# TXH-mercury/VALOR

Hardware: AMD Instinct MI355X
Metric: pretrain samples/sec (V+A+T clip) (higher is better)
Workload: dtype bf16

## Files before the change

valor_amd/csrc/gemm8q.hip:

```cpp
#include "gemm_common.h"
#include <stdlib.h>

#define HT_BYTES 16384
#define BUF_BYTES (4 * HT_BYTES)
#define OFF_A0 0
#define OFF_A1 HT_BYTES
#define OFF_B0 (2 * HT_BYTES)
#define OFF_B1 (3 * HT_BYTES)

template <bool KSLOW> struct FragSet;
template <> struct FragSet<false> { bf16x8_t f[4][2]; };
template <> struct FragSet<true> { TrPair f[4][2]; };
DEVINL bf16x8_t frag_of(const bf16x8_t& f) { return f; }
DEVINL bf16x8_t frag_of(const TrPair& t) { return tr_frag(t); }
DEVINL void mfma_acc(f32x4_t& c, bf16x8_t a, bf16x8_t b) { asm("v_mfma_f32_16x16x32_bf16 %0, %1, %2, %0" : "+a"(c) : "v"(a), "v"(b)); }
DEVINL void mfma_rowsum(f32x4_t& r0, f32x4_t& r1, bf16x8_t ones, bf16x8_t f0, bf16x8_t f1, bf16x8_t f2, bf16x8_t f3, int sel) {
    asm volatile("s_cmp_lt_i32 %7, 1\n\ts_cbranch_scc1 2f\n\ts_cmp_eq_u32 %7, 1\n\ts_cbranch_scc0 1f\n\t"
                 "v_mfma_f32_16x16x32_bf16 %0, %2, %3, %0\n\tv_mfma_f32_16x16x32_bf16 %1, %2, %4, %1\n\ts_branch 2f\n"
                 "1:\n\tv_mfma_f32_16x16x32_bf16 %0, %2, %5, %0\n\tv_mfma_f32_16x16x32_bf16 %1, %2, %6, %1\n"
                 "2:"
                 : "+v"(r0), "+v"(r1) : "v"(ones), "v"(f0), "v"(f1), "v"(f2), "v"(f3), "s"(sel) : "scc");
}
DEVINL void wait8(FragSet<false>&) { asm volatile("s_waitcnt lgkmcnt(0)" ::: "memory"); }
DEVINL void wait8(FragSet<true>& s) { tr_wait8(s.f); }
DEVINL void wait4(FragSet<false>&, int) { asm volatile("s_waitcnt lgkmcnt(0)" ::: "memory"); }
DEVINL void wait4(FragSet<true>& s, int kk) { tr_wait_4(s.f[0][kk], s.f[1][kk], s.f[2][kk], s.f[3][kk]); }

template <bool TA, bool TB>
__global__ __launch_bounds__(256) void gemm_8q_kernel(GemmArgs p) {
    typedef bf16_t T;
    constexpr int BK = 64;
    extern __shared__ __attribute__((aligned(16))) char smem[];

    const int tid = threadIdx.x;
    const int lane = tid & 63;
    const int wave = __builtin_amdgcn_readfirstlane(tid >> 6);
    const int wm = wave >> 1, wn = wave & 1;
    const int fr = lane & 15, fg = lane >> 4;

    const int tiles_n = (p.N + 255) >> 8;
    const int tiles_m = (p.M + 255) >> 8;
    int logical, slice = 0;
    if (p.kslices > 1) {
        const int ntiles = tiles_m * tiles_n;
        const int item = xcd_remap(blockIdx.x, ntiles * p.kslices);
        slice = item / ntiles;
        logical = item - slice * ntiles;
    } else {
        logical = xcd_remap(blockIdx.x, tiles_m * tiles_n);
    }
    int tm = logical / tiles_n, tn = logical - tm * tiles_n;
    if (p.raster_g > 0 && p.kslices <= 1) {
        const int G = p.raster_g, per = G * tiles_m;
        const int grp = logical / per, w = logical - grp * per;
        const int gw = min(G, tiles_n - grp * G);
        tm = w / gw;
        tn = grp * G + (w - tm * gw);
    }
    const int m0 = tm << 8, n0 = tn << 8;

    const int nk_total = p.K / BK;
    int ks_begin = 0, ks_end = nk_total;
    if (p.kslices > 1) {
        ks_begin = slice * p.ksteps_per_slice;
        ks_end = ks_begin + p.ksteps_per_slice;
        if (ks_end > nk_total) ks_end = nk_total;
        if (ks_begin > nk_total) ks_begin = nk_total;
    }
    const int k_first = ks_begin * BK;
    const int ntile = ks_end - ks_begin;

    f32x4_t acc[8][8];
#pragma unroll
    for (int i = 0; i < 8; ++i)
#pragma unroll
        for (int j = 0; j < 8; ++j) acc[i][j] = (f32x4_t){0.f, 0.f, 0.f, 0.f};

    const bool do_rs = TA && p.rowsum_out != nullptr && tn == 0;
    f32x4_t racc[2][2];
#pragma unroll
    for (int i = 0; i < 2; ++i)
#pragma unroll
        for (int j = 0; j < 2; ++j) racc[i][j] = (f32x4_t){0.f, 0.f, 0.f, 0.f};
    bf16x8_t ones = __builtin_bit_cast(bf16x8_t, (u32x4_t){0x3f803f80u, 0x3f803f80u, 0x3f803f80u, 0x3f803f80u});
    asm volatile("" : "+v"(ones));
    const int rs_sel = __builtin_amdgcn_readfirstlane(do_rs ? wn + 1 : 0);

    int oA[2][4], oB[2][4];
    int stepA, stepB;
    {
        const int ldA_b = (int)(p.lda * 2), ldB_b = (int)(p.ldb * 2);
#pragma unroll
        for (int hf = 0; hf < 2; ++hf)
#pragma unroll
            for (int i = 0; i < 4; ++i) {
                const int pc = wave * 4 + i;
                if constexpr (!TA) {
                    const int r = pc * 8 + (lane >> 3), c = (lane & 7) ^ ((lane >> 3) & 7);
                    oA[hf][i] = (m0 + hf * 128 + r) * ldA_b + (k_first + c * 8) * 2;
                } else {
                    const int k = pc * 4 + (lane >> 4), s = lane & 15;
                    const int ic = ((s - 2 * (k & 3) - 8 * ((k >> 3) & 1)) & 15) * 8;
                    oA[hf][i] = (k_first + k) * ldA_b + (m0 + hf * 128 + ic) * 2;
                }
                if constexpr (!TB) {
                    const int r = pc * 8 + (lane >> 3), c = (lane & 7) ^ ((lane >> 3) & 7);
                    oB[hf][i] = (n0 + hf * 128 + r) * ldB_b + (k_first + c * 8) * 2;
                } else {
                    const int k = pc * 4 + (lane >> 4), s = lane & 15;
                    const int ic = ((s - 2 * (k & 3) - 8 * ((k >> 3) & 1)) & 15) * 8;
                    oB[hf][i] = (k_first + k) * ldB_b + (n0 + hf * 128 + ic) * 2;
                }
            }
        stepA = TA ? BK * ldA_b : BK * 2;
        stepB = TB ? BK * ldB_b : BK * 2;
    }
    auto dmaA = [&](int hf, char* buf, int t, int i) {
        const rsrc_t rs = make_rsrc(p.A, t < ntile ? p.bytesA : 0u);
        glds16(rs, buf + (hf ? OFF_A1 : OFF_A0) + wave * 4096 + i * 1024, oA[hf][i]);
        oA[hf][i] += stepA; asm volatile("" : "+v"(oA[hf][i]));
    };
    auto dmaB = [&](int hf, char* buf, int t, int i) {
        const rsrc_t rs = make_rsrc(p.B, t < ntile ? p.bytesB : 0u);
        glds16(rs, buf + (hf ? OFF_B1 : OFF_B0) + wave * 4096 + i * 1024, oB[hf][i]);
        oB[hf][i] += stepB; asm volatile("" : "+v"(oB[hf][i]));
    };

    int trA[4], trB[4];
    {
        const int base = (8 * fg + (fr >> 2)) * 256 + 8 * (fr & 1);
        const int rot = 2 * (fr >> 2) + 8 * (fg & 1);
#pragma unroll
        for (int i = 0; i < 4; ++i) {
            trA[i] = base + 16 * ((2 * (wm * 4 + i) + ((fr >> 1) & 1) + rot) & 15);
            trB[i] = base + 16 * ((2 * (wn * 4 + i) + ((fr >> 1) & 1) + rot) & 15);
        }
    }
    auto rdA = [&](const char* img, FragSet<TA>& s, int mt, int kk) {
        if constexpr (TA) tr_issue(s.f[mt][kk], img + trA[mt] + kk * (32 * 256));
        else s.f[mt][kk] = read_frag<T>(img, wm * 64 + mt * 16 + fr, kk * 4 + fg);
    };
    auto rdB = [&](const char* img, FragSet<TB>& s, int nt, int kk) {
        if constexpr (TB) tr_issue(s.f[nt][kk], img + trB[nt] + kk * (32 * 256));
        else s.f[nt][kk] = read_frag<T>(img, wn * 64 + nt * 16 + fr, kk * 4 + fg);
    };
#define PIN() __builtin_amdgcn_sched_barrier(0)
    auto quadrant = [&](int mh, int nh, FragSet<TA>& sa, FragSet<TB>& sb, auto&& slot) __attribute__((always_inline)) {
#pragma unroll
        for (int kk = 0; kk < 2; ++kk)
#pragma unroll
            for (int mt = 0; mt < 4; ++mt)
#pragma unroll
                for (int nt = 0; nt < 4; ++nt) {
                    const int i = kk * 16 + mt * 4 + nt;
                    mfma_acc(acc[mh * 4 + mt][nh * 4 + nt], frag_of(sb.f[nt][kk]), frag_of(sa.f[mt][kk]));
                    slot(i);
                    PIN();
                }
    };
    auto rowsum = [&](int hh, FragSet<TA>& sa) __attribute__((always_inline)) {
        if constexpr (TA) {
#pragma unroll
            for (int kk = 0; kk < 2; ++kk)
                mfma_rowsum(racc[hh][0], racc[hh][1], ones, frag_of(sa.f[0][kk]), frag_of(sa.f[1][kk]), frag_of(sa.f[2][kk]), frag_of(sa.f[3][kk]), rs_sel);
            PIN();
        }
    };
#define PHASE_END()                                                                                               \
    do {                                                                                                          \
        asm volatile("s_waitcnt vmcnt(20)" ::: "memory");                                                         \
        __builtin_amdgcn_s_barrier();                                                                             \
        PIN();                                                                                                    \
    } while (0)

    FragSet<TA> fax, fay;
    FragSet<TB> fb0, fb1;
    if (ntile > 0) {
#pragma unroll
        for (int t = 0; t < 2; ++t) {
            char* const b = smem + t * BUF_BYTES;
#pragma unroll
            for (int i = 0; i < 4; ++i) dmaA(0, b, t, i);
#pragma unroll
            for (int i = 0; i < 4; ++i) dmaB(0, b, t, i);
#pragma unroll
            for (int i = 0; i < 4; ++i) dmaB(1, b, t, i);
#pragma unroll
            for (int i = 0; i < 4; ++i) dmaA(1, b, t, i);
        }
        PIN();
        PHASE_END();
#pragma unroll
        for (int i = 0; i < 8; ++i) rdA(smem + OFF_A0, fax, i & 3, i >> 2);
#pragma unroll
        for (int i = 0; i < 4; ++i) rdB(smem + OFF_B0, fb0, i, 0);
        PIN();
        wait8(fax); wait4(fb0, 0);
        __builtin_amdgcn_s_barrier();
        PIN();
        for (int rel = 0; rel < ntile; ++rel) {
            char* const cur = smem + (rel & 1) * BUF_BYTES;
            char* const nxt = smem + ((rel & 1) ^ 1) * BUF_BYTES;
            quadrant(0, 0, fax, fb0, [&](int i) {
                if (i < 4) rdB(cur + OFF_B0, fb0, i, 1);
                else if (i < 8) dmaA(0, cur, rel + 2, i - 4);
                else if (i == 15) { PIN(); wait4(fb0, 1); }
                else if (i >= 16 && i < 24) rdB(cur + OFF_B1, fb1, i & 3, (i - 16) >> 2);
            });
            rowsum(0, fax);
            PIN();
            wait8(fb1);
            PHASE_END();
            quadrant(0, 1, fax, fb1, [&](int i) {
                if (i < 8) rdA(cur + OFF_A1, fay, i & 3, i >> 2);
                else if (i < 16 && !(i & 1)) dmaB(0, cur, rel + 2, (i - 8) >> 1);
            });
            PIN();
            wait8(fay);
            PHASE_END();
            quadrant(1, 1, fay, fb1, [&](int i) {
                if (i < 4) rdA(nxt + OFF_A0, fax, i, 0);
                else if (i >= 8 && i < 16 && !(i & 1)) dmaB(1, cur, rel + 2, (i - 8) >> 1);
            });
            rowsum(1, fay);
            PIN();
            wait4(fax, 0);
            PHASE_END();
            quadrant(1, 0, fay, fb0, [&](int i) {
                if (i < 4) rdA(nxt + OFF_A0, fax, i, 1);
                else if (i >= 8 && i < 16 && !(i & 1)) dmaA(1, cur, rel + 2, (i - 8) >> 1);
                else if (i >= 16 && i < 20) rdB(nxt + OFF_B0, fb0, i - 16, 0);
            });
            PIN();
            wait4(fax, 1); wait4(fb0, 0);
            PHASE_END();
        }
    }
    asm volatile("s_nop 15\n\ts_nop 15\n\ts_waitcnt vmcnt(0)" ::: "memory");
    PIN();
    __syncthreads();
#undef PHASE_END
#undef PIN
    if (do_rs && fg == 0) {
#pragma unroll
        for (int hh = 0; hh < 2; ++hh)
#pragma unroll
            for (int i = 0; i < 2; ++i) {
                const int m = m0 + hh * 128 + wm * 64 + (2 * wn + i) * 16 + fr;
                if (m < p.M) {
                    if (p.kslices > 1) p.rowsum_ws[(int64_t)slice * p.M + m] = racc[hh][i][0];
                    else rowsum_store<T>(p, m, racc[hh][i][0]);
                }
            }
    }

    float* sC = (float*)smem;
    float* wsl = p.kslices > 1 ? p.ws + (int64_t)slice * p.M * p.N : nullptr;
    const f32x4_t bias0 = load_bias4<T>(p, n0 + (tid & 31) * 8), bias1 = load_bias4<T>(p, n0 + (tid & 31) * 8 + 4);
#pragma unroll
    for (int pass = 0; pass < 2; ++pass) {
        if (pass) __syncthreads();
#pragma unroll
        for (int mt = 0; mt < 4; ++mt)
#pragma unroll
            for (int ni = 0; ni < 8; ++ni) {
                const int ml = wm * 64 + mt * 16 + fr;
                const int ch = ((ni >> 2) * 32 + wn * 16 + (ni & 3) * 4 + fg) ^ (ml & 7);
                *(f32x4_t*)(sC + ml * 256 + ch * 4) = acc[pass * 4 + mt][ni];
            }
        __syncthreads();
#pragma unroll 2
        for (int it = 0; it < 16; ++it) {
            const int ml = it * 8 + (tid >> 5);
            const int c8 = tid & 31;
            const f32x4_t v0 = *(const f32x4_t*)(sC + ml * 256 + (((2 * c8) ^ (ml & 7)) << 2));
            const f32x4_t v1 = *(const f32x4_t*)(sC + ml * 256 + (((2 * c8 + 1) ^ (ml & 7)) << 2));
            const int m = m0 + pass * 128 + ml, n = n0 + c8 * 8;
            if (wsl) {
                splitk_store8(p, slice, m, n, v0, v1);
            } else {
                epilogue_store8<true, 0>(p, m, n, v0, v1, bias0, bias1);
            }
        }
    }
}

void launch_gemm_8q(hipStream_t st, int transA, int transB, const GemmArgs& p_in) {
    GemmArgs p = p_in;
    p.fast_epi = 0;
    p.raster_g = 0;
    p.st_mode = 0;
    const int tiles = ((p.M + 255) / 256) * ((p.N + 255) / 256);
    dim3 grid(tiles * (p.kslices > 1 ? p.kslices : 1));
    const size_t lds = 2 * BUF_BYTES;
#define VALOR_8Q_LAUNCH(TA_, TB_)                                                                               \
    do {                                                                                                        \
        static bool attr_set = false;                                                                           \
        if (!attr_set) {                                                                                        \
            hipFuncSetAttribute((const void*)gemm_8q_kernel<TA_, TB_>, hipFuncAttributeMaxDynamicSharedMemorySize, (int)lds); \
            attr_set = true;                                                                                    \
        }                                                                                                       \
        hipLaunchKernelGGL((gemm_8q_kernel<TA_, TB_>), grid, dim3(256), lds, st, p);                            \
    } while (0)
    if (transA && transB) VALOR_8Q_LAUNCH(true, true);
    else if (!transA && !transB) VALOR_8Q_LAUNCH(false, false);
    else if (!transA && transB) VALOR_8Q_LAUNCH(false, true);
    else VALOR_8Q_LAUNCH(true, false);
#undef VALOR_8Q_LAUNCH
}
```

Baseline: 580.6.

## Add slot-scheduled main loop for TA&&TB GEMM with finer LDS waits

For the transposed-A and transposed-B instantiation, replaces the quadrant/phase main loop with eight compile-time unrolled 16-MFMA slots. Each slot interleaves individual transposed LDS reads and DMA issues at fixed MFMA positions and uses partial lgkmcnt waits so older reads can be consumed while newer ones are still in flight. Global-load barriers are reduced to two per tile instead of four, and precomputed LDS addresses are ping-ponged between the two buffers. It also adds optional timestamp instrumentation and ablation macros, both off by default. The hand-counted waitcnt values carry a correctness risk if the instruction ordering shifts.

```diff
diff --git a/valor_amd/csrc/gemm8q.hip b/valor_amd/csrc/gemm8q.hip
--- a/valor_amd/csrc/gemm8q.hip
+++ b/valor_amd/csrc/gemm8q.hip
@@ -1,5 +1,6 @@
 #include "gemm_common.h"
 #include <stdlib.h>
+#include <type_traits>
 
 #define HT_BYTES 16384
 #define BUF_BYTES (4 * HT_BYTES)
@@ -26,9 +27,49 @@
 DEVINL void wait4(FragSet<false>&, int) { asm volatile("s_waitcnt lgkmcnt(0)" ::: "memory"); }
 DEVINL void wait4(FragSet<true>& s, int kk) { tr_wait_4(s.f[0][kk], s.f[1][kk], s.f[2][kk], s.f[3][kk]); }
 
+template <int NEWER> DEVINL void wait4_older(FragSet<true>& s, int kk) {
+    asm volatile("s_waitcnt lgkmcnt(%8)" : TR_TIE(s.f[0][kk]), TR_TIE(s.f[1][kk]), TR_TIE(s.f[2][kk]), TR_TIE(s.f[3][kk]) : "n"(NEWER));
+}
+
+template <int FIRST, int LAST, class F> DEVINL void static_for(F&& f) {
+    if constexpr (FIRST < LAST) {
+        f(std::integral_constant<int, FIRST>{});
+        static_for<FIRST + 1, LAST>(f);
+    }
+}
+template <int HT_OFF, int KK, int J> DEVINL void tr_read1(FragSet<true>& s, const uint32_t (&ad)[4]) {
+    if constexpr (J & 1) asm volatile("ds_read_b64_tr_b16 %0, %1 offset:%2" : "=v"(s.f[J >> 1][KK].hi) : "v"(ad[J >> 1]), "n"(HT_OFF + KK * (32 * 256) + 1024));
+    else asm volatile("ds_read_b64_tr_b16 %0, %1 offset:%2" : "=v"(s.f[J >> 1][KK].lo) : "v"(ad[J >> 1]), "n"(HT_OFF + KK * (32 * 256)));
+}
+
+#ifdef Q8_STAMP
+#define Q8_STAMP_TILE 5
+#define Q8_STAMP_BLOCKS 1024
+__device__ uint64_t q8_stamp_buf[Q8_STAMP_BLOCKS * 4 * 64];
+extern "C" int valor_gemm8q_read_stamps(void* host, int64_t bytes) {
+    if (bytes > (int64_t)sizeof(uint64_t) * Q8_STAMP_BLOCKS * 4 * 64) return VALOR_ERR_ARG;
+    return hipMemcpyFromSymbol(host, HIP_SYMBOL(q8_stamp_buf), (size_t)bytes, 0, hipMemcpyDeviceToHost) == hipSuccess ? 0 : VALOR_ERR_ARG;
+}
+#define Q8_AT(i) st_[i] = __builtin_amdgcn_s_memtime()
+#define Q8_HS(i) do { if (rel == Q8_STAMP_TILE) hs_[i] = __builtin_amdgcn_s_memtime(); __builtin_amdgcn_sched_barrier(0); } while (0)
+#else
+#define Q8_AT(i)
+#define Q8_HS(i)
+#endif
+#ifndef Q8_ABLATE
+#define Q8_ABLATE 0
+#endif
+
 template <bool TA, bool TB>
 __global__ __launch_bounds__(256) void gemm_8q_kernel(GemmArgs p) {
     typedef bf16_t T;
+    constexpr bool SLOTS = TA && TB;
+#ifdef Q8_STAMP
+    uint64_t st_[8] = {0, 0, 0, 0, 0, 0, 0, 0}, hs_[32];
+#pragma unroll
+    for (int i = 0; i < 32; ++i) hs_[i] = 0;
+    Q8_AT(0);
+#endif
     constexpr int BK = 64;
     extern __shared__ __attribute__((aligned(16))) char smem[];
 
@@ -173,8 +214,12 @@
         PIN();                                                                                                    \
     } while (0)
 
+#define LOOP_DMA(...) do { if constexpr (!(Q8_ABLATE & 1)) { __VA_ARGS__; } } while (0)
+#define LOOP_RD(...) do { if constexpr (!(Q8_ABLATE & 2)) { __VA_ARGS__; } } while (0)
+
     FragSet<TA> fax, fay;
     FragSet<TB> fb0, fb1;
+    if constexpr (!SLOTS) {
     if (ntile > 0) {
 #pragma unroll
         for (int t = 0; t < 2; ++t) {
@@ -236,11 +281,120 @@
             PHASE_END();
         }
     }
+    } else {
+    if (ntile > 0) {
+#define SLOT_END(s, tie, nfly)                                                                                    \
+    do {                                                                                                          \
+        Q8_HS(1 + 2 * (s));                                                                                       \
+        tie;                                                                                                      \
+        PIN();                                                                                                    \
+        if constexpr ((nfly) > 0) {                                                                               \
+            Q8_HS(17 + 2 * ((s) >> 1));                                                                           \
+            asm volatile("s_waitcnt vmcnt(%0)" ::"n"(nfly) : "memory");                                           \
+            Q8_HS(18 + 2 * ((s) >> 1));                                                                           \
+            __builtin_amdgcn_s_barrier();                                                                         \
+            PIN();                                                                                                \
+        }                                                                                                         \
+        Q8_HS(2 + 2 * (s));                                                                                       \
+    } while (0)
+#pragma unroll
+        for (int t = 0; t < 2; ++t) {
+            char* const b = smem + t * BUF_BYTES;
+#pragma unroll
+            for (int i = 0; i < 4; ++i) dmaA(0, b, t, i);
+#pragma unroll
+            for (int i = 0; i < 4; ++i) dmaB(0, b, t, i);
+#pragma unroll
+            for (int i = 0; i < 4; ++i) dmaB(1, b, t, i);
+#pragma unroll
+            for (int i = 0; i < 4; ++i) dmaA(1, b, t, i);
+        }
+        PIN();
+        asm volatile("s_waitcnt vmcnt(16)" ::: "memory");
+        __builtin_amdgcn_s_barrier();
+        PIN();
+#pragma unroll
+        for (int i = 0; i < 8; ++i) rdA(smem + OFF_A0, fax, i & 3, i >> 2);
+#pragma unroll
+        for (int i = 0; i < 8; ++i) rdB(smem + OFF_B0, fb0, i & 3, i >> 2);
+        PIN();
+        wait8(fax); wait8(fb0);
+        __builtin_amdgcn_s_barrier();
+        PIN();
+        Q8_AT(1);
+#ifdef Q8_STAMP
+        st_[6] = __builtin_amdgcn_s_memrealtime();
+#endif
+        uint32_t adA[4], adB[4], anA[4], anB[4];
+        int adelta = BUF_BYTES;
+#pragma unroll
+        for (int i = 0; i < 4; ++i) {
+            adA[i] = (uint32_t)(uintptr_t)LDS_PTR(smem) + trA[i];
+            adB[i] = (uint32_t)(uintptr_t)LDS_PTR(smem) + trB[i];
+            anA[i] = adA[i] + BUF_BYTES;
+            anB[i] = adB[i] + BUF_BYTES;
+        }
+        auto slot = [&](int mh, int nh, int kk, FragSet<true>& sa, FragSet<true>& sb, auto&& gap) __attribute__((always_inline)) {
+            static_for<0, 16>([&](auto ic) __attribute__((always_inline)) {
+                constexpr int i = decltype(ic)::value;
+                mfma_acc(acc[mh * 4 + (i >> 2)][nh * 4 + (i & 3)], frag_of(sb.f[i & 3][kk]), frag_of(sa.f[i >> 2][kk]));
+                gap(ic);
+                PIN();
+            });
+        };
+        for (int rel = 0; rel < ntile; ++rel) {
+            char* const cur = smem + (rel & 1) * BUF_BYTES;
+            char* const nxt = smem + ((rel & 1) ^ 1) * BUF_BYTES;
+            Q8_HS(0);
+            {
+#define GAP(d0, d1, ...)                                                                                          \
+    [&](auto ic) __attribute__((always_inline)) {                                                                 \
+        constexpr int i = decltype(ic)::value;                                                                    \
+        LOOP_RD(__VA_ARGS__);                                                                                     \
+        if constexpr (i == 9) LOOP_DMA(d0);                                                                       \
+        if constexpr (i == 13) LOOP_DMA(d1);                                                                      \
+    }
+                slot(0, 0, 0, fax, fb0, GAP(dmaA(0, cur, rel + 2, 0), dmaA(0, cur, rel + 2, 1), if constexpr (i < 8) tr_read1<OFF_B1, 0, (i & 7)>(fb1, adB); else tr_read1<OFF_B1, 1, (i & 7)>(fb1, adB)));
+                SLOT_END(0, (void)0, 0);
+                slot(0, 0, 1, fax, fb0, GAP(dmaA(0, cur, rel + 2, 2), dmaA(0, cur, rel + 2, 3), if constexpr (i < 8) tr_read1<OFF_A1, 0, (i & 7)>(fay, adA)));
+                rowsum(0, fax);
+                SLOT_END(1, (wait4_older<8>(fb1, 0), wait4_older<8>(fb1, 1)), 0);
+                slot(0, 1, 0, fax, fb1, GAP(dmaB(0, cur, rel + 2, 0), dmaB(0, cur, rel + 2, 1), if constexpr (i < 8) tr_read1<OFF_A1, 1, (i & 7)>(fay, adA)));
+                SLOT_END(2, wait4_older<8>(fay, 0), 0);
+                slot(0, 1, 1, fax, fb1, GAP(dmaB(0, cur, rel + 2, 2), dmaB(0, cur, rel + 2, 3), (void)0));
+                SLOT_END(3, wait4(fay, 1), 16);
+                slot(1, 0, 0, fay, fb0, GAP(dmaB(1, cur, rel + 2, 0), dmaB(1, cur, rel + 2, 1), if constexpr (i < 8) tr_read1<OFF_A0, 0, (i & 7)>(fax, anA)));
+                SLOT_END(4, (void)0, 0);
+                slot(1, 0, 1, fay, fb0, GAP(dmaB(1, cur, rel + 2, 2), dmaB(1, cur, rel + 2, 3), if constexpr (i < 8) tr_read1<OFF_A0, 1, (i & 7)>(fax, anA)));
+                rowsum(1, fay);
+                SLOT_END(5, wait4_older<8>(fax, 0), 0);
+                slot(1, 1, 0, fay, fb1, GAP(dmaA(1, cur, rel + 2, 0), dmaA(1, cur, rel + 2, 1), if constexpr (i < 8) tr_read1<OFF_B0, 0, (i & 7)>(fb0, anB); else tr_read1<OFF_B0, 1, (i & 7)>(fb0, anB)));
+                SLOT_END(6, wait4_older<15>(fax, 1), 0);
+                slot(1, 1, 1, fay, fb1, [&](auto ic) __attribute__((always_inline)) {
+                    constexpr int i = decltype(ic)::value;
+                    if constexpr (i < 2) { adA[2 * i] += adelta; adA[2 * i + 1] += adelta; }
+                    else if constexpr (i < 4) { adB[2 * i - 4] += adelta; adB[2 * i - 3] += adelta; }
+                    else if constexpr (i < 6) { anA[2 * i - 8] -= adelta; anA[2 * i - 7] -= adelta; }
+                    else if constexpr (i < 8) { anB[2 * i - 12] -= adelta; anB[2 * i - 11] -= adelta; }
+                    if constexpr (i == 8) { adelta = -adelta; asm volatile("" : "+s"(adelta)); }
+                    if constexpr (i == 9) LOOP_DMA(dmaA(1, cur, rel + 2, 2));
+                    if constexpr (i == 13) LOOP_DMA(dmaA(1, cur, rel + 2, 3));
+                });
+                SLOT_END(7, wait8(fb0), 16);
+#undef GAP
+            }
+        }
+#undef SLOT_END
+    }
+    }
+#ifdef Q8_STAMP
+    st_[7] = __builtin_amdgcn_s_memrealtime();
+#endif
+    Q8_AT(2);
     asm volatile("s_nop 15\n\ts_nop 15\n\ts_waitcnt vmcnt(0)" ::: "memory");
     PIN();
     __syncthreads();
-#undef PHASE_END
-#undef PIN
+    Q8_AT(3);
     if (do_rs && fg == 0) {
 #pragma unroll
         for (int hh = 0; hh < 2; ++hh)
@@ -282,7 +436,26 @@
                 epilogue_store8<true, 0>(p, m, n, v0, v1, bias0, bias1);
             }
         }
-    }
+#ifdef Q8_STAMP
+        asm volatile("s_waitcnt vmcnt(0)" ::: "memory");
+        st_[4 + pass] = __builtin_amdgcn_s_memtime();
+#endif
+    }
+#ifdef Q8_STAMP
+    if (lane == 0 && blockIdx.x < Q8_STAMP_BLOCKS) {
+        uint64_t* o = q8_stamp_buf + ((int64_t)blockIdx.x * 4 + wave) * 64;
+        for (int i = 0; i < 8; ++i) o[i] = st_[i];
+        o[8] = __builtin_amdgcn_s_getreg((31 << 11) | 4);
+        o[9] = __builtin_amdgcn_s_getreg((31 << 11) | 20);
+        o[10] = ntile;
+        o[11] = SLOTS;
+        for (int i = 0; i < 32; ++i) o[16 + i] = hs_[i];
+    }
+#endif
+#undef PHASE_END
+#undef LOOP_DMA
+#undef LOOP_RD
+#undef PIN
 }
 
 void launch_gemm_8q(hipStream_t st, int transA, int transB, const GemmArgs& p_in) {
@@ -293,7 +466,7 @@
     const int tiles = ((p.M + 255) / 256) * ((p.N + 255) / 256);
     dim3 grid(tiles * (p.kslices > 1 ? p.kslices : 1));
     const size_t lds = 2 * BUF_BYTES;
-#define VALOR_8Q_LAUNCH(TA_, TB_)                                                                               \
+#define VALOR_8Q_LAUNCH(TA_, TB_)                                                                             \
     do {                                                                                                        \
         static bool attr_set = false;                                                                           \
         if (!attr_set) {                                                                                        \
```

New measurement: 587.2, median of 6. 1.01x the previous value.
